# ende76/brotli-rs

Hardware: AMD Instinct MI355X
Metric: decompressed MB/s (whole node), alice29x4096 batch (higher is better)
Workload: dtype u8; 1 GPU; 4096 x alice29.txt.compressed per GPU; streams_per_gpu=4096

## Files before the change

brotli-rs_amd/build.py:

```python
import os
import re
import subprocess
import sys

PKG = os.path.dirname(os.path.abspath(__file__))
ROOT = os.path.dirname(PKG)
CSRC = os.path.join(PKG, "csrc")
LIB_PATH = os.path.join(PKG, "libbrx.so")
HIPCC = os.environ.get("HIPCC", "/opt/rocm/bin/hipcc")
SOURCES = ["brx_kernels.hip", "brx_kernels_l1.hip", "brx_kernels_l2.hip", "brx_kernels_l3.hip", "brx_kernels_l4.hip", "brx_kernels_s.hip", "brx_gen.hip", "brx_util.hip", "brx_tiles.hip", "brx_digest.hip", "brx_index.hip", "brx_api.cpp", "brx_node.cpp"]
DEPS = SOURCES + ["brx_device.h", "brx_layout.h", "brx_tiles.h", "brx_digest.h", "brx_index.h", "brx_internal.h", "brx_plan.h", "brx_small.h", "brx_hot.S", "brx_lens.S", os.path.join("..", "host", "brx_walk.cpp"), os.path.join("..", "..", "include", "brx.h"),
                  os.path.join("..", "tables", "dictionary.bin"), os.path.join("..", "tables", "context_lut.bin"),
                  os.path.join("..", "tables", "transforms.bin"), os.path.join("..", "tables", "gen_header.bin"), os.path.join("..", "build.py")]


def _stale():
    if not os.path.exists(LIB_PATH):
        return True
    t = os.path.getmtime(LIB_PATH)
    return any(os.path.getmtime(os.path.join(CSRC, d)) > t for d in DEPS)


def build_library(force=False, verbose=False):
    if not force and not _stale():
        return LIB_PATH
    import fcntl
    with open(os.path.join(PKG, ".build.lock"), "w") as lock:
        fcntl.flock(lock, fcntl.LOCK_EX)
        if not force and not _stale():
            return LIB_PATH
        return _build_locked(verbose)


def _build_locked(verbose):
    if not os.path.exists(HIPCC):
        if os.path.exists(LIB_PATH):
            return LIB_PATH
        raise RuntimeError("hipcc not found at %s and no prebuilt libbrx.so" % HIPCC)
    gen = os.path.join(CSRC, "_gen", "brx_tables_gen.h")
    subprocess.check_call([sys.executable, os.path.join(ROOT, "tools", "bin2h.py"), gen, "BRX", "static const"])
    prof = ["-DBRX_PROF"] if os.environ.get("BRX_PROF") == "1" else []
    if os.environ.get("BRX_NO_SPEC") == "1":
        prof.append("-DBRX_NO_SPEC")
    if os.environ.get("BRX_PIN_NOPS"):
        prof.append("-DPIN_NOPS=%d" % int(os.environ["BRX_PIN_NOPS"]))
    extra = ["-D" + d for d in os.environ.get("BRX_DEFS", "").split()]
    prof += extra
    instances = [("" if k == 0 else "_l%d" % k, "-DBRX_LEVEL=%d" % k) for k in range(5)] + [("_s", "-DBRX_SMALL")]

    def emit(src, name, defs):
        txt = subprocess.check_output(["cpp", "-P", "-x", "assembler-with-cpp"] + defs + [os.path.join(CSRC, src)]).decode()
        assert ")BRXASM" not in txt and "%" not in txt and "{" not in txt and "$" not in txt
        if src == "brx_hot.S":
            if "-DBRX_WIN_SGPR" in defs:
                txt = txt.replace(".L", ".LS_")
            macros = re.findall(r"^\s*\.macro\s+(\w+)", txt, flags=re.M)
            txt += "".join(".purgem %s\n" % m for m in macros)
        else:
            txt = re.sub(r"@(\d+)@", r"%\1", txt).replace(".Lls_", ".Lls%=_")
        with open(os.path.join(CSRC, "_gen", name), "w") as f:
            f.write("// generated from %s by build.py -- do not edit\n" % src)
            f.write('R"BRXASM(\n' + txt + ')BRXASM"\n')

    for suffix, level in instances:
        if suffix != "_s":
            emit("brx_hot.S", "brx_hot_asm%s.h" % suffix, prof + [level])
            emit("brx_hot.S", "brx_hot_asm_sw%s.h" % suffix, prof + [level, "-DBRX_WIN_SGPR"])
        emit("brx_lens.S", "brx_lens_asm%s.h" % suffix, [level])
    cmd = [HIPCC, "--offload-arch=gfx950", "-O3", "-std=c++17", "-fPIC", "-shared", "-Wno-comment"]
    if os.environ.get("BRX_BRINGUP") == "1" or os.environ.get("BRX_PROF") == "1":
        cmd.append("-DBRX_BRINGUP")
    cmd += extra + [os.path.join(CSRC, s) for s in SOURCES]
    tmp = "%s.tmp.%d" % (LIB_PATH, os.getpid())
    cmd += ["-ldl", "-lpthread", "-o", tmp]
    if verbose:
        print(" ".join(cmd))
    subprocess.check_call(cmd, cwd=CSRC)
    os.replace(tmp, LIB_PATH)
    walk = os.path.join(PKG, "brx_walk")
    subprocess.check_call(["g++", "-O2", "-std=c++17", os.path.join(PKG, "host", "brx_walk.cpp"), "-o", walk + ".tmp", "-L", PKG,
                           "-lbrx", "-Wl,-rpath,$ORIGIN", "-Wl,-rpath,/opt/rocm/lib", "-L/opt/rocm/lib", "-lamdhip64"])
    os.replace(walk + ".tmp", walk)
    return LIB_PATH


if __name__ == "__main__":
    print(build_library(force="--force" in sys.argv, verbose=True))
```

brotli-rs_amd/csrc/brx_kernels.hip:

```cpp
#include <hip/hip_runtime.h>

#include "brx_device.h"

#ifdef BRX_SMALL
#define BRX_INST _s
#elif BRX_LEVEL == 0
#define BRX_INST
#else
#define BRX_INST BRX_L_PASTE(_l, BRX_LEVEL)
#endif
#define BRX_NAME(stem) BRX_L_PASTE(stem, BRX_INST)
#define BRX_STR_(x) #x
#define BRX_STR(x) BRX_STR_(x)
#define BRX_GEN_H(stem) BRX_STR(_gen/BRX_NAME(stem).h)

typedef unsigned char u8;
typedef unsigned short u16;
typedef unsigned int u32;
typedef unsigned long long u64;

#define RMASK (BRX_RING_BYTES - 1u)
#define TM_BYTES (BRX_TM_WORDS * 4u)

enum {
// ... 250 lines not shown
        d.chunkA = in_load_chunk(d, d.cbase);
        d.chunkB = in_load_chunk(d, d.cbase + 64u);
    }
    while (w >= d.cbase + 128u) {
        d.chunkA = d.chunkB;
        d.cbase += 64u;
        d.chunkB = in_load_chunk(d, d.cbase + 64u);
    }
    u32 k = w - d.cbase;
    return k < 64u ? rdl(d.chunkA, k) : rdl(d.chunkB, k - 64u);
}
FI void in_seek(Dec &d, u64 bitpos) {
    d.bitpos = bitpos;
    d.ww = (u32)(bitpos >> 5);
    u64 lo = in_word(d, d.ww);
    u64 hi = in_word(d, d.ww + 1u);
    d.win = lo | (hi << 32);
}
FI u64 in_remaining(const Dec &d) { return d.bitend - d.bitpos; }
FI u32 in_peek_raw(const Dec &d) { return (u32)(d.win >> (d.bitpos & 31u)); }
FI void in_consume(Dec &d, u32 n) {
    d.bitpos += n;
    if ((u32)(d.bitpos >> 5) != d.ww) {
        d.ww += 1u;
        u64 hi = in_word(d, d.ww + 1u);
        d.win = (d.win >> 32) | (hi << 32);
    }
}
FI bool in_bits(Dec &d, u32 n, u32 &v) {
    if (in_remaining(d) < n) return false;
    v = n ? (in_peek_raw(d) & ((1u << n) - 1u)) : 0u;
    in_consume(d, n);
    return true;
}
FI u32 in_byte_tail(Dec &d) {
    u32 k = (u32)(d.bitpos & 7u);
    u32 v = 0;
    if (k) in_bits(d, 8u - k, v);
    return v;
}

#define ST_STARTED 33
#define ST_ISLAST 34
#define ST_MLEN 35
#define ST_IACTAB 36
#define ST_POOL 38
#define ST_MIRROR 40
#define ST_PAUSE_AT 43
#define ST_IN_LOW 45
#define ST_SPEC 47
#define ST_NEED 42
#define SEG_NEED_HEADER 100u
#define SEG_PAUSED 101u
#define HC_WHOLE 0u
#define HC_START 1u
#define HC_RESUME_R0 2u
#define HC_RESUME_R1 3u
#define HC_RESUME_R2 4u
#define HC_RESUME_R1_WHOLE 5u
#define HC_TO_END 8u
#define HC_CONTINUE 200u
#define MBW_ASM 31
#define MBW_MBLEFT 32
#define MBW_INS 33
#define MBW_CPY 34
#define MBW_IZ 35
#define MBW_DIST 36
#define MBW_DISTBAD 37
#define MBW_EXIT 38
#define BRX_END_MARGIN 5u
#ifndef BRX_SPEC_CK_DWORDS
#define BRX_SPEC_CK_DWORDS 64u
#endif
#ifndef BRX_SPEC_CK_MIN_DWORDS
#define BRX_SPEC_CK_MIN_DWORDS 1024u
#endif
#define MBW_WSAFE 39

#ifndef BRX_SMALL
FI void put64(Lds &s, u32 i, u64 v) { s.st[i] = (u32)v; s.st[i + 1u] = (u32)(v >> 32); }
FI u64 get64(const Lds &s, u32 i) { return (u64)rfl(s.st[i]) | ((u64)rfl(s.st[i + 1u]) << 32); }
FI void dec_store(const Dec &d, Lds &s) {
    {
        put64(s, 0, (u64)(uintptr_t)d.in_words); s.st[2] = d.w_end; put64(s, 3, d.bitpos); put64(s, 5, d.bitend);
        put64(s, 7, (u64)(uintptr_t)d.out); s.st[9] = d.cap; s.st[10] = d.pos; s.st[11] = d.a; s.st[12] = d.vfl;
        s.st[13] = d.window; s.st[14] = d.dist0; s.st[15] = d.dist1; s.st[16] = d.dist2; s.st[17] = d.dist3;
        s.st[18] = d.lds_top; s.st[19] = d.scr_top; put64(s, 20, (u64)(uintptr_t)d.scratch); s.st[22] = d.needed;
        put64(s, 23, (u64)(uintptr_t)d.t_dict); put64(s, 25, (u64)(uintptr_t)d.t_xforms);
        put64(s, 27, (u64)(uintptr_t)d.t_lut); put64(s, 29, d.wd); put64(s, 31, d.wd_limit);
        put64(s, ST_POOL, (u64)(uintptr_t)d.pool);
        put64(s, ST_MIRROR, (u64)(uintptr_t)d.mirror);
    }
}
FI void dec_load(Dec &d, const Lds &s) {
    d.lane = threadIdx.x;
    d.in_words = (const u32 *)(uintptr_t)get64(s, 0); d.w_end = rfl(s.st[2]);
    d.bitend = get64(s, 5);
    d.out = (u8 *)(uintptr_t)get64(s, 7); d.cap = rfl(s.st[9]);
    d.out_rsrc = __builtin_amdgcn_make_buffer_rsrc(d.out, 0, d.cap, 0x00020000);
    d.mirror = (u8 *)(uintptr_t)get64(s, ST_MIRROR);
    d.out2_rsrc = __builtin_amdgcn_make_buffer_rsrc(d.mirror, 0, d.mirror ? d.cap : 0u, 0x00020000);
    d.pos = rfl(s.st[10]); d.a = rfl(s.st[11]);
    d.vfl = rfl(s.st[12]); d.window = rfl(s.st[13]);
    d.dist0 = rfl(s.st[14]); d.dist1 = rfl(s.st[15]); d.dist2 = rfl(s.st[16]); d.dist3 = rfl(s.st[17]);
    d.lds_top = rfl(s.st[18]); d.scr_top = rfl(s.st[19]); d.scratch = (u32 *)(uintptr_t)get64(s, 20);
    d.needed = rfl(s.st[22]);
    d.t_dict = (const u8 *)(uintptr_t)get64(s, 23); d.t_xforms = (const BrxTransform *)(uintptr_t)get64(s, 25);
    d.t_lut = (const u32 *)(uintptr_t)get64(s, 27); d.wd = get64(s, 29); d.wd_limit = get64(s, 31);
    d.pool = (const BrxSlabPool *)(uintptr_t)get64(s, ST_POOL);
    d.need_cur = 0u; d.need_peak = 0u;
    d.cbase = 0xffffff00u;
    d.chunkA = 0; d.chunkB = 0;
    in_seek(d, get64(s, 3));
}

FI void dec_load_in(Dec &d, const Lds &s) {
    d.lane = threadIdx.x;
    d.in_words = (const u32 *)(uintptr_t)get64(s, 0); d.w_end = rfl(s.st[2]);
    d.bitend = get64(s, 5);
    d.lds_top = rfl(s.st[18]); d.scr_top = rfl(s.st[19]); d.scratch = (u32 *)(uintptr_t)get64(s, 20);
    d.pool = (const BrxSlabPool *)(uintptr_t)get64(s, ST_POOL);
    d.need_cur = 0u; d.need_peak = 0u;
    d.cbase = 0xffffff00u;
    d.chunkA = 0; d.chunkB = 0;
    in_seek(d, get64(s, 3));
}
FI void dec_store_in(const Dec &d, Lds &s) {
    put64(s, 3, d.bitpos);
    s.st[18] = d.lds_top; s.st[19] = d.scr_top; put64(s, 20, (u64)(uintptr_t)d.scratch);
    s.st[ST_NEED] = d.need_peak;
}

#endif

#define BRX_HDR_WORDS 17u
#define BRX_HDR_INFO 16u
#define BRX_DIST_UNFIT 0xc0000000u
template <bool INL, bool WIDE> FI u32 decode_sym_as(Dec &d, const Lds &s, u32 h, u32 &sym) {
    u32 hv = tm_ld32<INL>(d, s, h + (d.lane & 31u));
    u32 h0 = rdl(hv, BRX_HDR_INFO);
    u32 kind = h0 & 3u;
    if (kind == 0u) return LK_NONE;
    if (kind == 1u) {
        sym = h0 >> 16;
        if (WIDE && sym == 0xffffu) sym = rfl(tm_ld32<INL>(d, s, h + 13u));
        return LK_OK;
    }
    u64 rem = in_remaining(d);
    u32 peek = in_peek_raw(d) & 0x7fffu;
    if (rem < 15u) peek &= (1u << (u32)rem) - 1u;
    u32 v = __brev(peek) >> 17;
    u64 m = ballot(((v << 16) | 0xffffu) < hv) & 0xfffeull;
    if (m == 0ull) {
        u32 maxlen = (h0 >> 8) & 0xffu;
        return rem >= (u64)(maxlen + 1u) ? LK_NONE : LK_EOF;
    }
    u32 L = (u32)__builtin_ctzll(m);
    if ((u64)L > rem) return LK_EOF;
    u32 base = rdl(hv, L);
    u32 idx = ((v >> (15u - L)) + base) & 0xffffu;
    sym = WIDE ? rfl(tm_ld32<INL>(d, s, h + BRX_HDR_WORDS + idx)) : rfl(tm_ld16<INL>(d, s, (h + BRX_HDR_WORDS) * 2u + idx));
    in_consume(d, L);
    return LK_OK;
}
FI u32 decode_sym(Dec &d, const Lds &s, u32 h, u32 &sym) {
    if (h < BRX_TM_WORDS) return decode_sym_as<true, false>(d, s, h, sym);
    return decode_sym_as<false, false>(d, s, h, sym);
}
FI u32 decode_sym_wide(Dec &d, const Lds &s, u32 h, u32 &sym) {
    if (h < BRX_TM_WORDS) return decode_sym_as<true, true>(d, s, h, sym);
    return decode_sym_as<false, true>(d, s, h, sym);
}

#ifdef BRX_SMALL
FI u32 hb_word(Dec &d, u32 w) {
    const u32 v = rfl(w < 64u ? rdl(d.chunkA, w & 63u) : rdl(d.chunkB, w & 63u));
    return w < 128u ? v : 0u;
}
#else
FI u32 hb_word(Dec &d, u32 w) {
    const u32 v = in_word(d, w);
    return w == d.hb_lastw ? v & d.hb_lastmask : v;
}
#endif
FI void hb_begin(Dec &d) {
    const u32 w = (u32)(d.bitpos >> 5), sh = (u32)d.bitpos & 31u;
    d.hb_lastw = (u32)((d.bitend - 1ull) >> 5);
    const u32 r = (u32)d.bitend & 31u;
    d.hb_lastmask = r ? (1u << r) - 1u : 0xffffffffu;
    const u64 lo = hb_word(d, w), hi = hb_word(d, w + 1u);
    d.win = (lo | (hi << 32)) >> sh;
    d.nav = 64u - sh;
    d.ww = w + 2u;
}
FI u64 hb_pos(const Dec &d) { return 32ull * d.ww - d.nav; }
FI bool hb_over(const Dec &d) { return hb_pos(d) > d.bitend; }
FI u32 hb_peek(const Dec &d) { return (u32)d.win; }
FI void hb_skip(Dec &d, u32 n) {
    d.win >>= n;
    d.nav -= n;
    if (d.nav < 32u) {
        d.win |= (u64)hb_word(d, d.ww) << d.nav;
        d.nav += 32u;
        d.ww += 1u;
    }
}
FI u32 hb_bits(Dec &d, u32 n) {
    const u32 v = hb_peek(d) & ((1u << n) - 1u);
    hb_skip(d, n);
    return v;
}

FI u32 row_scan_add(u32 x) {
    x += (u32)__builtin_amdgcn_update_dpp(0, (int)x, 0x111, 0xf, 0xf, true);
    x += (u32)__builtin_amdgcn_update_dpp(0, (int)x, 0x112, 0xf, 0xf, true);
    x += (u32)__builtin_amdgcn_update_dpp(0, (int)x, 0x114, 0xf, 0xf, true);
    x += (u32)__builtin_amdgcn_update_dpp(0, (int)x, 0x118, 0xf, 0xf, true);
    return x;
}
FI u32 lanes_below(u64 m) { return __builtin_amdgcn_mbcnt_hi((u32)(m >> 32), __builtin_amdgcn_mbcnt_lo((u32)m, 0u)); }

FI u32 emit_code_header(Dec &d, Lds &s, u32 cnt, const bool wide, u32 &off) {
    const u32 lane = d.lane, L = lane & 15u;
    const u32 c = (lane - 1u) < 15u ? cnt : 0u;
    const u32 lim = row_scan_add(c << (15u - L));
    const u32 offi = row_scan_add(c);
    off = offi - c;
    const u32 base = off - ((lim >> (15u - L)) - c);
    const u32 nnz = rdl(offi, 15);
    const u32 maxlen = 63u - (u32)__builtin_clzll(ballot(c != 0u) | 1ull);
    const u32 h = tm_alloc(d, BRX_HDR_WORDS + (wide ? nnz : ((nnz + 1u) >> 1)));
    const u32 w = lane == 0u ? 0u : lane == BRX_HDR_INFO ? (2u | (maxlen << 8) | (nnz << 16)) : (lim << 16) | (base & 0xffffu);
    if (h < BRX_TM_WORDS) { if (lane < BRX_HDR_WORDS) tm_st32<true>(d, s, h + lane, w); }
    else { if (lane < BRX_HDR_WORDS) tm_st32<false>(d, s, h + lane, w); }
    return h;
}
FI void code_put_symbol(const Dec &d, Lds &s, u32 h, const bool wide, bool on, u32 slot, u32 sym) {
    if (wide) {
        if (h < BRX_TM_WORDS) { if (on) tm_st32<true>(d, s, h + BRX_HDR_WORDS + slot, sym); }
        else { if (on) tm_st32<false>(d, s, h + BRX_HDR_WORDS + slot, sym); }
    } else {
        if (h < BRX_TM_WORDS) { if (on) tm_st16<true>(d, s, (h + BRX_HDR_WORDS) * 2u + slot, sym); }
        else { if (on) tm_st16<false>(d, s, (h + BRX_HDR_WORDS) * 2u + slot, sym); }
    }
}

FI u32 build_code(Dec &d, Lds &s, u32 n, const bool wide = false) {
    const u32 lane = d.lane;
    u32 *const cnt = (u32 *)&s.lens[704];
    if (lane < 16u) cnt[lane] = 0u;
    const u32 nch = (n + 63u) >> 6;
    for (u32 c = 0; c < nch; c++) {
        const u32 i = c * 64u + lane;
        const u32 my = i < n ? s.lens[i] : 0u;
        __hip_atomic_fetch_add(&cnt[my], 1u, __ATOMIC_RELAXED, __HIP_MEMORY_SCOPE_WORKGROUP);
    }
    u32 off;
    const u32 h = emit_code_header(d, s, cnt[lane & 15u], wide, off);
    if (lane < 16u) cnt[lane] = off;
    for (u32 c = 0; c < nch; c++) {
        const u32 i = c * 64u + lane;
        const u32 my = i < n ? s.lens[i] : 0u;
        if (ballot(my != 0u) == 0ull) continue;
        const u64 b0 = ballot((my & 1u) != 0u), b1 = ballot((my & 2u) != 0u), b2 = ballot((my & 4u) != 0u), b3 = ballot((my & 8u) != 0u);
        u64 eq = (my & 1u) ? b0 : ~b0;
        eq &= (my & 2u) ? b1 : ~b1;
        eq &= (my & 4u) ? b2 : ~b2;
        eq &= (my & 8u) ? b3 : ~b3;
        const u32 slot = cnt[my] + lanes_below(eq);
        code_put_symbol(d, s, h, wide, my != 0u, slot, i);
        __hip_atomic_fetch_add(&cnt[my], 1u, __ATOMIC_RELAXED, __HIP_MEMORY_SCOPE_WORKGROUP);
    }
    return h;
}

FI u32 build_simple(Dec &d, Lds &s, u32 nsym, u32 k0, u32 k1, u32 k2, u32 k3, const bool wide) {
    if (nsym < 3u) k2 = 0xffffffffu;
    if (nsym < 4u) k3 = 0xffffffffu;
    u32 t;
#define BRX_CSWAP(a, b) do { t = a < b ? a : b; b = a < b ? b : a; a = t; } while (0)
    BRX_CSWAP(k0, k1); BRX_CSWAP(k2, k3); BRX_CSWAP(k0, k2); BRX_CSWAP(k1, k3); BRX_CSWAP(k1, k2);
#undef BRX_CSWAP
    const u32 lane = d.lane;
    const u32 cnt = (u32)((k0 >> 16) == lane) + (u32)((k1 >> 16) == lane) + (u32)((k2 >> 16) == lane) + (u32)((k3 >> 16) == lane);
    u32 off;
    const u32 h = emit_code_header(d, s, cnt, wide, off);
    const u32 mine = lane == 0u ? k0 : lane == 1u ? k1 : lane == 2u ? k2 : k3;
    code_put_symbol(d, s, h, wide, lane < nsym, lane, mine & 0xffffu);
    return h;
}

FI u32 build_single(Dec &d, Lds &s, u32 sym) {
    u32 h = tm_alloc(d, BRX_HDR_WORDS);
    u32 w = d.lane == BRX_HDR_INFO ? (1u | (sym << 16)) : 0u;
    if (h < BRX_TM_WORDS) { if (d.lane < BRX_HDR_WORDS) tm_st32<true>(d, s, h + d.lane, w); }
    else { if (d.lane < BRX_HDR_WORDS) tm_st32<false>(d, s, h + d.lane, w); }
    return h;
}

FI void lens_clear(const Dec &d, Lds &s, u32 n) {
    for (u32 i = d.lane * 4u; i < n; i += 256u) *(u32 *)&s.lens[i] = 0u;
}

FI u32 read_complex_lens(Dec &d, Lds &s, u32 hskip, u32 alphabet) {
    PT_BEGIN(pt);
    const u32 lane = d.lane;
    u32 clv = 0;
    u32 sum = 0, nonzero = 0, single = 0;
    bool parallel_done = false;
#ifndef BRX_NO_PAR_CLCODE
    {
        const u32 w0 = hb_word(d, d.ww), w1 = hb_word(d, d.ww + 1u);
        const u64 lo = d.nav < 64u ? (d.win | ((u64)w0 << d.nav)) : d.win;
        const u64 hi = ((u64)w0 >> (64u - d.nav)) | ((u64)w1 << (d.nav - 32u));
        const u32 p = (u32)((lo >> lane) | (lane ? hi << ((64u - lane) & 63u) : 0ull)) & 15u;
        const u32 len = (p & 1u) == 0u ? 2u : (p & 2u) == 0u ? 2u : (p & 4u) == 0u ? 3u : 4u;
        const u32 val = (p & 1u) == 0u ? ((p & 2u) ? 3u : 0u) : (p & 2u) == 0u ? 4u : (p & 4u) == 0u ? 2u : ((p & 8u) ? 5u : 1u);
        const u32 lv = len | (val << 4);
        const u32 nx = lane + len;
        const u32 j1 = nx < 63u ? nx : 63u;
        const u32 j2 = (u32)__shfl((int)j1, (int)j1), j4 = (u32)__shfl((int)j2, (int)j2), j8 = (u32)__shfl((int)j4, (int)j4),
                  j16 = (u32)__shfl((int)j8, (int)j8);
        u32 pos = 0;
        {
            const u32 t1 = (u32)__shfl((int)j1, (int)pos); pos = (lane & 1u) ? t1 : pos;
            const u32 t2 = (u32)__shfl((int)j2, (int)pos); pos = (lane & 2u) ? t2 : pos;
            const u32 t4 = (u32)__shfl((int)j4, (int)pos); pos = (lane & 4u) ? t4 : pos;
            const u32 t8 = (u32)__shfl((int)j8, (int)pos); pos = (lane & 8u) ? t8 : pos;
            const u32 t16 = (u32)__shfl((int)j16, (int)pos); pos = (lane & 16u) ? t16 : pos;
        }
        const u32 mine = (u32)__shfl((int)lv, (int)pos);
        const u32 n = 18u - hskip;
        const u32 myval = lane < n ? mine >> 4 : 0u, mylen = mine & 15u;
        const u32 space = myval ? 32u >> myval : 0u;
        const u32 sc = row_scan_add(space);
        const u32 cum = lane >= 16u ? sc + rdl(sc, 15) : sc;
        const u64 hit = ballot(lane < n && cum >= 32u);
        const u32 count = hit ? (u32)__builtin_ctzll(hit) + 1u : n;
        const u32 last_end = rdl(pos + mylen, count - 1u);
        if (last_end <= 60u) {
            sum = rdl(cum, count - 1u);
            const u64 nzm = ballot(lane < count && myval != 0u);
            nonzero = (u32)__builtin_popcountll(nzm);
            const u32 inv = lane == 0u ? 4u : lane <= 4u ? lane - 1u : lane == 5u ? 5u : lane == 6u ? 7u : lane == 16u ? 8u : lane == 17u ? 6u : lane + 2u;
            const u32 k = inv - hskip;
            const u32 got = (u32)__shfl((int)myval, (int)(k & 63u));
            clv = (lane < 18u && k < count) ? got : 0u;
            if (nzm) {
                const u32 kl = 63u - (u32)__builtin_clzll(nzm), il = hskip + kl;
                single = il < 4u ? il + 1u : il == 4u ? 0u : il == 5u ? 5u : il == 6u ? 17u : il == 7u ? 6u : il == 8u ? 16u : il - 2u;
            }
            hb_skip(d, last_end > 32u ? 32u : last_end);
            if (last_end > 32u) hb_skip(d, last_end - 32u);
            if (sum > 32u) return ST_CODE_LENGTHS_CHECKSUM;
            parallel_done = true;
        }
    }
#endif
    for (u32 i = hskip; i < 18u && !parallel_done; i++) {
        const u32 p = hb_peek(d) & 15u;
        u32 len, val;
        if ((p & 1u) == 0u) { len = 2; val = (p & 2u) ? 3u : 0u; }
        else if ((p & 2u) == 0u) { len = 2; val = 4u; }
        else if ((p & 4u) == 0u) { len = 3; val = 2u; }
        else { len = 4; val = (p & 8u) ? 5u : 1u; }
        hb_skip(d, len);
        if (val) {
            const u32 symi = i < 4u ? i + 1u : i == 4u ? 0u : i == 5u ? 5u : i == 6u ? 17u : i == 7u ? 6u : i == 8u ? 16u : i - 2u;
            clv = wrl(val, symi, clv);
            sum += 32u >> val;
            nonzero++;
            single = symi;
            if (sum == 32u) break;
            if (sum > 32u) return ST_CODE_LENGTHS_CHECKSUM;
        }
    }
    if (nonzero == 0u) return ST_NO_CODE_LENGTH;
    if (nonzero >= 2u && sum < 32u) return ST_CODE_LENGTHS_CHECKSUM;

    u32 cltab = 0;
    if (nonzero >= 2u) {
        const u32 l = lane < 18u ? clv : 0u;
        const u64 b0 = ballot((l & 1u) != 0u), b1 = ballot((l & 2u) != 0u), b2 = ballot((l & 4u) != 0u);
        u64 eq = (l & 1u) ? b0 : ~b0;
        eq &= (l & 2u) ? b1 : ~b1;
        eq &= (l & 4u) ? b2 : ~b2;
        const u32 rank = lanes_below(eq);
        u32 code = 0, mycode = 0;
        for (u32 k = 1; k <= 5u; k++) {
            if (l == k) mycode = code + rank;
            const u64 mk = ((k & 1u) ? b0 : ~b0) & ((k & 2u) ? b1 : ~b1) & ((k & 4u) ? b2 : ~b2);
            code = (code + (u32)__builtin_popcountll(mk)) << 1;
        }
        const u32 rev = l ? __brev(mycode) >> (32u - l) : 0u;
        u64 todo = ballot(l != 0u);
        while (todo) {
            const u32 sy = (u32)__builtin_ctzll(todo);
            todo &= todo - 1ull;
            const u32 ls = rdl(l, sy), rs = rdl(rev, sy);
            if ((lane & ((1u << ls) - 1u)) == rs) cltab = (sy << 4) | ls;
        }
    }

    lens_clear(d, s, alphabet);
    PT_ADD(7, pt);
    u32 total = 0, i = 0, nz = 0;
    u32 last_symbol = 0xffu, last_repeat = 0, last_nz = 8;
    u32 cur = 0;
    bool dirty = false;
#define BRX_LENS_FLUSH(base_) do { if (dirty) s.lens[(base_) + lane] = (u8)cur; cur = 0u; dirty = false; } while (0)
    if (nonzero >= 2u) {
        u32 stat, nz_a, i_a, dirty_a, cur_a, vt0, vt1;
        u64 win = (u64)rfl((u32)d.win) | ((u64)rfl((u32)(d.win >> 32)) << 32);
        u32 nav = rfl(d.nav), ww = rfl(d.ww), cbase = rfl(d.cbase), cha = d.chunkA, chb = d.chunkB;
        asm volatile(
#include BRX_GEN_H(brx_lens_asm)
            : "=s"(stat), "=s"(nz_a), "=s"(i_a), "=s"(dirty_a), "+s"(win), "+s"(nav), "+s"(ww), "+s"(cbase), "+v"(cha), "+v"(chb),
              "=&v"(cur_a), "=&v"(vt0), "=&v"(vt1)
            : "s"(alphabet), "s"(d.w_end), "s"(d.hb_lastw), "s"(d.hb_lastmask), "s"((u64)(uintptr_t)d.in_words), "v"(cltab), "v"(lane)
            : "memory", "vcc", "scc", "s60", "s61", "s62", "s63", "s64", "s65", "s66", "s67", "s68", "s69", "s70", "s71", "s72", "s73",
              "s74", "s75", "s76", "s77", "s78", "s79", "s80", "s81", "s82", "s83", "s84", "s85", "s86", "s87", "s88", "s89", "s90");
        d.win = win; d.nav = nav; d.ww = ww; d.cbase = cbase; d.chunkA = cha; d.chunkB = chb;
        if (dirty_a) s.lens[((i_a - 1u) & ~63u) + lane] = (u8)cur_a;
        PT_ADD(8, pt);
        if (stat) return stat;
        if (nz_a < 2u) return ST_LESS_THAN_TWO_NONZERO;
        return ST_OK;
    }
    while (i < alphabet) {
        u32 sym;
        if (nonzero == 1u) {
            sym = single;
        } else {
            const u32 e = rdl(cltab, hb_peek(d) & 31u);
            sym = e >> 4;
            hb_skip(d, e & 15u);
        }
        if (sym <= 15u) {
            cur = wrl(sym, i & 63u, cur);
            i++;
            last_symbol = sym;
            last_repeat = 0;
            if (sym) {
                dirty = true;
                nz++;
                last_nz = sym;
                total += 32768u >> sym;
                if (total == 32768u) break;
                if (total > 32768u) return ST_CODE_LENGTHS_CHECKSUM;
            }
            if ((i & 63u) == 0u) BRX_LENS_FLUSH(i - 64u);
        } else if (sym == 16u) {
            const u32 v = hb_bits(d, 2);
            u32 add, new_repeat;
            if (last_symbol == 16u && last_repeat) {
                new_repeat = 4u * (last_repeat - 2u) + v + 3u;
                add = new_repeat - last_repeat;
            } else {
                new_repeat = 3u + v;
                add = new_repeat;
            }
            if (i + add > alphabet) return ST_PARSE_COMPLEX_LENGTHS;
            nz += add;
            total += add * (32768u >> last_nz);
            for (u32 left = add; left != 0u;) {
                const u32 a0 = i & 63u, k = left < 64u - a0 ? left : 64u - a0;
                cur = (lane - a0) < k ? last_nz : cur;
                dirty = true;
                i += k;
                left -= k;
                if ((i & 63u) == 0u) BRX_LENS_FLUSH(i - 64u);
            }
            if (total == 32768u) break;
            if (total > 32768u) return ST_CODE_LENGTHS_CHECKSUM;
            last_repeat = new_repeat;
            last_symbol = 16u;
        } else {
            const u32 v = hb_bits(d, 3);
            u32 ni;
            if (last_symbol == 17u && last_repeat) {
                const u32 new_repeat = 8u * (last_repeat - 2u) + v + 3u;
                ni = i + (new_repeat - last_repeat);
                last_repeat = new_repeat;
            } else {
                last_repeat = 3u + v;
                ni = i + last_repeat;
            }
            if (ni > alphabet) return ST_PARSE_COMPLEX_LENGTHS;
            if ((ni >> 6) != (i >> 6)) BRX_LENS_FLUSH(i & ~63u);
            i = ni;
            last_symbol = 17u;
        }
    }
    BRX_LENS_FLUSH((i - 1u) & ~63u);
#undef BRX_LENS_FLUSH
    PT_ADD(8, pt);
    if (nz < 2u) return ST_LESS_THAN_TWO_NONZERO;
    return ST_OK;
}

FI u32 read_prefix_code(Dec &d, Lds &s, u32 alphabet, u32 &h, const bool wide = false) {
    PT_BEGIN(pt);
    const u32 kind = hb_bits(d, 2);
    if (kind == 1u) {
        const u32 bit_width = 32u - (u32)__builtin_clz(alphabet - 1u);
        const u32 nsym = hb_bits(d, 2) + 1u;
        u32 s0 = 0, s1 = 0, s2 = 0, s3 = 0;
        s0 = hb_bits(d, bit_width);
        if (s0 >= alphabet) return ST_INVALID_SYMBOL;
        if (nsym > 1u) {
            s1 = hb_bits(d, bit_width);
            if (s1 >= alphabet) return ST_INVALID_SYMBOL;
        }
        if (nsym > 2u) {
            s2 = hb_bits(d, bit_width);
            if (s2 >= alphabet) return ST_INVALID_SYMBOL;
        }
        if (nsym > 3u) {
            s3 = hb_bits(d, bit_width);
            if (s3 >= alphabet) return ST_INVALID_SYMBOL;
        }
        if (nsym > 1u && s0 == s1) return ST_INVALID_SYMBOL;
        if (nsym > 2u && (s0 == s2 || s1 == s2)) return ST_INVALID_SYMBOL;
        if (nsym > 3u && (s0 == s3 || s1 == s3 || s2 == s3)) return ST_INVALID_SYMBOL;
        u32 tree_select = 0;
        if (nsym == 4u) tree_select = hb_bits(d, 1);
        if (nsym == 1u) {
            h = build_single(d, s, s0);
            PT_ADD(6, pt);
            return ST_OK;
        }
        u32 l0, l1, l2, l3;
        if (nsym == 2u) { l0 = 1; l1 = 1; l2 = 0; l3 = 0; }
        else if (nsym == 3u) { l0 = 1; l1 = 2; l2 = 2; l3 = 0; }
        else if (!tree_select) { l0 = l1 = l2 = l3 = 2; }
        else { l0 = 1; l1 = 2; l2 = 3; l3 = 3; }
        h = build_simple(d, s, nsym, (l0 << 16) | s0, (l1 << 16) | s1, (l2 << 16) | s2, (l3 << 16) | s3, wide);
        PT_ADD(6, pt);
        return ST_OK;
    }
    const u32 rc = read_complex_lens(d, s, kind, alphabet);
    if (rc) return rc;
    PT_BEGIN(pb);
    h = build_code(d, s, alphabet, wide);
    PT_ADD(9, pb);
    return ST_OK;
}

FI void ring_put(const Dec &d, Lds &s, bool on, u32 vpos, u32 byte) {
    u8 *p = on ? &s.ring[vpos & RMASK] : &s.trash[d.lane];
    *p = (u8)byte;
}
#define OUT_STORE128(q, off) do { const u32 off_ = (off); __builtin_amdgcn_raw_buffer_store_b128((q), d.out_rsrc, off_, 0, 0); \
                                  __builtin_amdgcn_raw_buffer_store_b128((q), d.out2_rsrc, off_, 0, 0); } while (0)
#define OUT_STORE8(b, off) do { const u32 off_ = (off); __builtin_amdgcn_raw_buffer_store_b8((u8)(b), d.out_rsrc, off_, 0, 0); \
                                __builtin_amdgcn_raw_buffer_store_b8((u8)(b), d.out2_rsrc, off_, 0, 0); } while (0)
FI void flush_range(Dec &d, const Lds &s, u32 v0, u32 v1) {
    const u32 u0 = (v0 + 15u) >> 4, u1 = v1 >> 4;
    for (u32 ub = u0; ub < u1; ub += 64u) {
        u32 u = ub + d.lane;
        typedef u32 u32x4 __attribute__((ext_vector_type(4)));
        u32x4 q = *(const u32x4 *)&s.ring[(u * 16u) & RMASK];
        u32 off = u < u1 ? u * 16u - d.a : 0xffffffffu;
        OUT_STORE128(q, off);
    }
    if (v0 & 15u) {
        u32 e = u0 * 16u < v1 ? u0 * 16u : v1;
        u32 v = v0 + d.lane;
        u32 b = s.ring[v & RMASK];
        OUT_STORE8(b, v < e ? v - d.a : 0xffffffffu);
    }
    if ((v1 & 15u) && u1 * 16u >= v0 && u1 >= u0) {
        u32 v = u1 * 16u + d.lane;
        u32 b = s.ring[v & RMASK];
        OUT_STORE8(b, v < v1 ? v - d.a : 0xffffffffu);
    }
    d.vfl = v1;
}
FI void maybe_flush(Dec &d, const Lds &s) {
    u32 vpos = d.pos + d.a;
    for (;;) {
        u32 blk_end = (d.vfl & ~(BRX_FLUSH_BLOCK - 1u)) + BRX_FLUSH_BLOCK;
        if (vpos < blk_end + BRX_FLUSH_LAG) break;
        flush_range(d, s, d.vfl, blk_end);
    }
}
FI bool out_room(Dec &d, u32 n) {
    if ((u64)d.pos + n > (u64)d.cap) {
        d.needed = (u64)d.pos + n > 0xffffffffull ? 0xffffffffu : d.pos + n;
        return false;
    }
    return true;
}
FI void ctx_bytes(const Dec &d, const Lds &s, u32 &p1, u32 &p2) {
    u32 v = d.pos + d.a;
    u32 b1 = s.ring[(v - 1u) & RMASK], b2 = s.ring[(v - 2u) & RMASK];
    p1 = d.pos >= 1u ? rfl(b1) : 0u;
    p2 = d.pos >= 2u ? rfl(b2) : 0u;
}

FI u32 copy_fetch(const Dec &d, const Lds &s, u32 back_max, u32 back_min, u32 back) {
    if (back_max <= BRX_RING_BYTES) return s.ring[(d.pos - back + d.a) & RMASK];
    if (back_min > BRX_RING_BYTES) return __builtin_amdgcn_raw_buffer_load_b8(d.out_rsrc, d.pos - back, 0, 0);
    u32 bn = s.ring[(d.pos - back + d.a) & RMASK];
    u32 bf = __builtin_amdgcn_raw_buffer_load_b8(d.out_rsrc, d.pos - back, 0, 0);
    return back <= BRX_RING_BYTES ? bn : bf;
}

typedef u32 u32x4 __attribute__((ext_vector_type(4)));
FI void bulk_copy_1k(Dec &d, Lds &s, u32 de) {
    const u32 vdst = d.pos + d.a + 16u * d.lane;
    u32x4 q;
    if (de <= BRX_RING_BYTES) {
        const u32 r = vdst - de;
        if ((de & 3u) == 0u) {
            q.x = *(const u32 *)&s.ring[r & RMASK];
            q.y = *(const u32 *)&s.ring[(r + 4u) & RMASK];
            q.z = *(const u32 *)&s.ring[(r + 8u) & RMASK];
            q.w = *(const u32 *)&s.ring[(r + 12u) & RMASK];
        } else {
            u32 w[4];
            _Pragma("unroll") for (u32 k = 0; k < 4u; k++) {
                u32 b0 = s.ring[(r + 4u * k) & RMASK], b1 = s.ring[(r + 4u * k + 1u) & RMASK];
                u32 b2 = s.ring[(r + 4u * k + 2u) & RMASK], b3 = s.ring[(r + 4u * k + 3u) & RMASK];
                w[k] = b0 | (b1 << 8) | (b2 << 16) | (b3 << 24);
            }
            q.x = w[0]; q.y = w[1]; q.z = w[2]; q.w = w[3];
        }
    } else {
        q = __builtin_amdgcn_raw_buffer_load_b128(d.out_rsrc, d.pos - de + 16u * d.lane, 0, 0);
    }
    *(u32x4 *)&s.ring[vdst & RMASK] = q;
    d.pos += 1024u;
}

#ifndef BRX_FILL_AUX
#define BRX_FILL_AUX 0
#endif
FI void periodic_fill(Dec &d, Lds &s, u32 P, u32 nblocks) {
    flush_range(d, s, d.vfl, d.pos + d.a);
    const u32 base = d.pos - P + d.a;
    u32 o = (16u * d.lane) % P;
    const u32 step = 1024u % P;
    {
        u32x4 q = *(const u32x4 *)&s.ring[(base + o) & RMASK];
        u32 off = d.pos + 16u * d.lane;
        if (step == 0u) {
            if (d.mirror == nullptr) {
                for (u32 k = 0; k < nblocks; k++) { __builtin_amdgcn_raw_buffer_store_b128(q, d.out_rsrc, off, 0, BRX_FILL_AUX); off += 1024u; }
            } else {
                for (u32 k = 0; k < nblocks; k++) { OUT_STORE128(q, off); off += 1024u; }
            }
        } else {
            const bool both = d.mirror != nullptr;
            for (u32 k = 0; k < nblocks; k++) {
                o += step;
                o = o >= P ? o - P : o;
                const u32x4 qn = *(const u32x4 *)&s.ring[(base + o) & RMASK];
                __builtin_amdgcn_raw_buffer_store_b128(q, d.out_rsrc, off, 0, BRX_FILL_AUX);
                if (both) __builtin_amdgcn_raw_buffer_store_b128(q, d.out2_rsrc, off, 0, 0);
                off += 1024u;
                q = qn;
            }
        }
        d.pos += nblocks << 10;
    }
    d.vfl = d.pos + d.a;
    static_assert(BRX_RING_BYTES == 2048u, "periodic_fill re-seeds two 1 KiB blocks");
    if (nblocks >= 2u) {
        const u32 o1 = o >= step ? o - step : o + P - step;
        const u32 o0 = o1 >= step ? o1 - step : o1 + P - step;
        const u32x4 q0 = *(const u32x4 *)&s.ring[(base + o0) & RMASK];
        const u32x4 q1 = *(const u32x4 *)&s.ring[(base + o1) & RMASK];
        const u32 off = d.pos - BRX_RING_BYTES + 16u * d.lane;
        *(u32x4 *)&s.ring[(off + d.a) & RMASK] = q0;
        *(u32x4 *)&s.ring[(off + 1024u + d.a) & RMASK] = q1;
        return;
    }
    __builtin_amdgcn_s_waitcnt(0x0F70);
    for (u32 j = 0; j < BRX_RING_BYTES / 1024u; j++) {
        const u32 off = d.pos - BRX_RING_BYTES + 1024u * j + 16u * d.lane;
        const u32x4 q = __builtin_amdgcn_raw_buffer_load_b128(d.out_rsrc, off, 0, 0);
        *(u32x4 *)&s.ring[(off + d.a) & RMASK] = q;
    }
}

FI void direct_far_copy(Dec &d, Lds &s, u32 de, u32 nblocks) {
    flush_range(d, s, d.vfl, d.pos + d.a);
    for (u32 k = 0; k < nblocks; k++) {
        if (de < 16384u) __builtin_amdgcn_s_waitcnt(0x0F70);
        const u32 src = d.pos - de + 16u * d.lane, dst = d.pos + 16u * d.lane;
        const u32x4 q0 = __builtin_amdgcn_raw_buffer_load_b128(d.out_rsrc, src, 0, 0);
        const u32x4 q1 = __builtin_amdgcn_raw_buffer_load_b128(d.out_rsrc, src + 1024u, 0, 0);
        const u32x4 q2 = __builtin_amdgcn_raw_buffer_load_b128(d.out_rsrc, src + 2048u, 0, 0);
        const u32x4 q3 = __builtin_amdgcn_raw_buffer_load_b128(d.out_rsrc, src + 3072u, 0, 0);
        OUT_STORE128(q0, dst);
        OUT_STORE128(q1, dst + 1024u);
        OUT_STORE128(q2, dst + 2048u);
        OUT_STORE128(q3, dst + 3072u);
        d.pos += 4096u;
    }
    d.vfl = d.pos + d.a;
    __builtin_amdgcn_s_waitcnt(0x0F70);
    for (u32 j = 0; j < BRX_RING_BYTES / 1024u; j++) {
        const u32 off = d.pos - BRX_RING_BYTES + 1024u * j + 16u * d.lane;
        const u32x4 q = __builtin_amdgcn_raw_buffer_load_b128(d.out_rsrc, off, 0, 0);
        *(u32x4 *)&s.ring[(off + d.a) & RMASK] = q;
    }
}

FI void window_copy(Dec &d, Lds &s, u32 dist, u32 len, u32 &p1, u32 &p2) {
    u32 done = 0, de = dist;
    bool bulk_used = false;
    const u32 g16 = dist & (0u - dist) & 15u ? (dist & (0u - dist) & 15u) : 16u;
    const u32 P16 = dist * (16u / g16);
    while (done < len) {
        const u32 rem = len - done;
        if (dist < len && rem >= 8192u && P16 <= 1024u && done + dist >= P16 && ((d.pos + d.a) & 15u) == 0u) {
            const u32 nb = rem >> 10;
            periodic_fill(d, s, P16, nb);
            done += nb << 10;
            bulk_used = true;
// ... 1428 lines not shown
```

brotli-rs_amd/csrc/brx_lens.S:

```
#include "brx_layout.h"
#define LDS_LENS BRX_L_LENS
#define WIN s[60:61]
#define WINLO s60
#define NAV s62
#define WW s63
#define IPOS s64
#define TOT s65
#define NZ s66
#define LNZ s67
#define LSYM s68
#define LREP s69
#define ALPHA s70
#define CBASE s71
#define WEND s72
#define LASTW s73
#define LMASK s74
#define ENT s75
#define SYM s76
#define LEN s77
#define T0 s78
#define T1 s79
#define PAIR s[80:81]
#define PLO s80
#define PHI s81
#define T2 s82
#define T3 s83
#define LINK s[84:85]
#define INW s[86:87]
#define STAT s88
#define DIRTY s89
#define LEFT s90
#define VCHA @8@
#define VCHB @9@
#define VCUR @10@
#define VT0 @11@
#define VT1 @12@
#define VCLTAB @18@
#define VLANE @19@

    s_mov_b64 WIN, @4@
    s_mov_b32 NAV, @5@
    s_mov_b32 WW, @6@
    s_mov_b32 CBASE, @7@
    s_mov_b32 ALPHA, @13@
    s_mov_b32 WEND, @14@
    s_mov_b32 LASTW, @15@
    s_mov_b32 LMASK, @16@
    s_mov_b64 INW, @17@
    s_mov_b32 IPOS, 0
    s_mov_b32 TOT, 0
    s_mov_b32 NZ, 0
    s_mov_b32 LNZ, 8
    s_mov_b32 LSYM, 0xff
    s_mov_b32 LREP, 0
    s_mov_b32 DIRTY, 0
    s_mov_b32 STAT, 0
    v_mov_b32 VCUR, 0
.Lls_sym:
    s_cmp_ge_u32 IPOS, ALPHA
    s_cbranch_scc1 .Lls_done
    s_and_b32 T0, WINLO, 31
    v_readlane_b32 ENT, VCLTAB, T0
    s_and_b32 LEN, ENT, 15
    s_lshr_b32 SYM, ENT, 4
    s_lshr_b64 WIN, WIN, LEN
    s_sub_u32 NAV, NAV, LEN
    s_cmp_lt_u32 NAV, 32
    s_cbranch_scc0 .Lls_have
    s_call_b64 LINK, .Lls_refill
.Lls_have:
    s_cmp_gt_u32 SYM, 15
    s_cbranch_scc1 .Lls_special
    s_and_b32 T0, IPOS, 63
    v_mov_b32 VT0, SYM
    v_cmp_eq_u32 vcc, T0, VLANE
    v_cndmask_b32 VCUR, VCUR, VT0, vcc
    s_add_u32 IPOS, IPOS, 1
    s_mov_b32 LSYM, SYM
    s_mov_b32 LREP, 0
    s_cmp_eq_u32 SYM, 0
    s_cbranch_scc1 .Lls_chunk
    s_mov_b32 DIRTY, 1
    s_add_u32 NZ, NZ, 1
    s_mov_b32 LNZ, SYM
    s_lshr_b32 T1, 0x8000, SYM
    s_add_u32 TOT, TOT, T1
    s_cmp_ge_u32 TOT, 0x8000
    s_cbranch_scc1 .Lls_total
.Lls_chunk:
    s_and_b32 T0, IPOS, 63
    s_cmp_lg_u32 T0, 0
    s_cbranch_scc1 .Lls_sym
    s_sub_u32 T0, IPOS, 64
    s_call_b64 LINK, .Lls_flush
    s_branch .Lls_sym
.Lls_total:
    s_cmp_eq_u32 TOT, 0x8000
    s_cbranch_scc1 .Lls_done
    s_mov_b32 STAT, 1
    s_branch .Lls_done
.Lls_special:
    s_cmp_eq_u32 SYM, 16
    s_cbranch_scc1 .Lls_rep
    s_and_b32 T0, WINLO, 7
    s_lshr_b64 WIN, WIN, 3
    s_sub_u32 NAV, NAV, 3
    s_cmp_lt_u32 NAV, 32
    s_cbranch_scc0 .Lls_z_have
    s_call_b64 LINK, .Lls_refill
.Lls_z_have:
    s_cmp_eq_u32 LSYM, 17
    s_cselect_b32 T1, LREP, 0
    s_cmp_eq_u32 T1, 0
    s_cbranch_scc1 .Lls_z_fresh
    s_sub_u32 T2, T1, 2
    s_lshl_b32 T2, T2, 3
    s_add_u32 T2, T2, T0
    s_add_u32 T2, T2, 3
    s_sub_u32 T3, T2, T1
    s_mov_b32 LREP, T2
    s_branch .Lls_z_go
.Lls_z_fresh:
    s_add_u32 T3, T0, 3
    s_mov_b32 LREP, T3
.Lls_z_go:
    s_mov_b32 LSYM, 17
    s_add_u32 T2, IPOS, T3
    s_cmp_gt_u32 T2, ALPHA
    s_cbranch_scc1 .Lls_err_parse
    s_xor_b32 T0, T2, IPOS
    s_cmp_lt_u32 T0, 64
    s_cbranch_scc1 .Lls_z_same
    s_and_b32 T0, IPOS, 0xffffffc0
    s_mov_b32 LEFT, T2
    s_call_b64 LINK, .Lls_flush
    s_mov_b32 T2, LEFT
.Lls_z_same:
    s_mov_b32 IPOS, T2
    s_branch .Lls_sym
.Lls_rep:
    s_and_b32 T0, WINLO, 3
    s_lshr_b64 WIN, WIN, 2
    s_sub_u32 NAV, NAV, 2
    s_cmp_lt_u32 NAV, 32
    s_cbranch_scc0 .Lls_r_have
    s_call_b64 LINK, .Lls_refill
.Lls_r_have:
    s_cmp_eq_u32 LSYM, 16
    s_cselect_b32 T1, LREP, 0
    s_cmp_eq_u32 T1, 0
    s_cbranch_scc1 .Lls_r_fresh
    s_sub_u32 T2, T1, 2
    s_lshl_b32 T2, T2, 2
    s_add_u32 T2, T2, T0
    s_add_u32 T2, T2, 3
    s_sub_u32 LEFT, T2, T1
    s_branch .Lls_r_go
.Lls_r_fresh:
    s_add_u32 T2, T0, 3
    s_mov_b32 LEFT, T2
.Lls_r_go:
    s_add_u32 T3, IPOS, LEFT
    s_cmp_gt_u32 T3, ALPHA
    s_cbranch_scc1 .Lls_err_parse
    s_add_u32 NZ, NZ, LEFT
    s_lshr_b32 T3, 0x8000, LNZ
    s_mul_i32 T3, T3, LEFT
    s_add_u32 TOT, TOT, T3
    s_mov_b32 LREP, T2
    s_mov_b32 LSYM, 16
    v_mov_b32 VT1, LNZ
.Lls_r_fill:
    s_and_b32 T0, IPOS, 63
    s_sub_u32 T1, 64, T0
    s_min_u32 T1, T1, LEFT
    v_subrev_u32 VT0, T0, VLANE
    v_cmp_gt_u32 vcc, T1, VT0
    v_cndmask_b32 VCUR, VCUR, VT1, vcc
    s_mov_b32 DIRTY, 1
    s_add_u32 IPOS, IPOS, T1
    s_sub_u32 LEFT, LEFT, T1
    s_and_b32 T0, IPOS, 63
    s_cmp_lg_u32 T0, 0
    s_cbranch_scc1 .Lls_r_next
    s_sub_u32 T0, IPOS, 64
    s_call_b64 LINK, .Lls_flush
    v_mov_b32 VT1, LNZ
.Lls_r_next:
    s_cmp_lg_u32 LEFT, 0
    s_cbranch_scc1 .Lls_r_fill
    s_cmp_ge_u32 TOT, 0x8000
    s_cbranch_scc1 .Lls_total
    s_branch .Lls_sym
.Lls_err_parse:
    s_mov_b32 STAT, 18
    s_branch .Lls_done

.Lls_flush:
    s_cmp_eq_u32 DIRTY, 0
    s_cbranch_scc1 .Lls_flush_empty
    v_add_u32 VT0, T0, VLANE
    ds_write_b8 VT0, VCUR offset:LDS_LENS
.Lls_flush_empty:
    v_mov_b32 VCUR, 0
    s_mov_b32 DIRTY, 0
    s_setpc_b64 LINK

.Lls_refill:
    s_sub_u32 T1, WW, CBASE
    s_cmp_lt_u32 T1, 128
    s_cbranch_scc1 .Lls_rf_staged
    s_waitcnt vmcnt(0)
    v_mov_b32 VCHA, VCHB
    s_add_u32 CBASE, CBASE, 64
    s_add_u32 T1, CBASE, 64
    v_add_u32 VT0, T1, VLANE
    v_cmp_gt_u32 vcc, WEND, VT0
    s_sub_u32 T2, WEND, 1
    v_min_u32 VT1, T2, VT0
    v_lshlrev_b32 VT1, 2, VT1
    global_load_dword VCHB, VT1, INW
    s_waitcnt vmcnt(0)
    v_cndmask_b32 VCHB, 0, VCHB, vcc
    s_sub_u32 T1, WW, CBASE
.Lls_rf_staged:
    s_cmp_lt_u32 T1, 64
    s_cbranch_scc0 .Lls_rf_b
    v_readlane_b32 PLO, VCHA, T1
    s_branch .Lls_rf_have
.Lls_rf_b:
    v_readlane_b32 PLO, VCHB, T1
.Lls_rf_have:
    s_cmp_lt_u32 WW, WEND
    s_cselect_b32 PLO, PLO, 0
    s_cmp_eq_u32 WW, LASTW
    s_cselect_b32 T2, LMASK, -1
    s_and_b32 PLO, PLO, T2
    s_mov_b32 PHI, 0
    s_lshl_b64 PAIR, PAIR, NAV
    s_or_b64 WIN, WIN, PAIR
    s_add_u32 NAV, NAV, 32
    s_add_u32 WW, WW, 1
    s_setpc_b64 LINK

.Lls_done:
    s_mov_b32 @0@, STAT
    s_mov_b32 @1@, NZ
    s_mov_b32 @2@, IPOS
    s_mov_b32 @3@, DIRTY
    s_mov_b64 @4@, WIN
    s_mov_b32 @5@, NAV
    s_mov_b32 @6@, WW
    s_mov_b32 @7@, CBASE
```

Measured before the change: 75820 MB/s.

## Decode complex code-length symbols in parallel across wavefront lanes before serial fallback

```diff
diff --git a/brotli-rs_amd/build.py b/brotli-rs_amd/build.py
--- a/brotli-rs_amd/build.py
+++ b/brotli-rs_amd/build.py
@@ -9,7 +9,7 @@
 LIB_PATH = os.path.join(PKG, "libbrx.so")
 HIPCC = os.environ.get("HIPCC", "/opt/rocm/bin/hipcc")
 SOURCES = ["brx_kernels.hip", "brx_kernels_l1.hip", "brx_kernels_l2.hip", "brx_kernels_l3.hip", "brx_kernels_l4.hip", "brx_kernels_s.hip", "brx_gen.hip", "brx_util.hip", "brx_tiles.hip", "brx_digest.hip", "brx_index.hip", "brx_api.cpp", "brx_node.cpp"]
-DEPS = SOURCES + ["brx_device.h", "brx_layout.h", "brx_tiles.h", "brx_digest.h", "brx_index.h", "brx_internal.h", "brx_plan.h", "brx_small.h", "brx_hot.S", "brx_lens.S", os.path.join("..", "host", "brx_walk.cpp"), os.path.join("..", "..", "include", "brx.h"),
+DEPS = SOURCES + ["brx_device.h", "brx_layout.h", "brx_tiles.h", "brx_digest.h", "brx_index.h", "brx_internal.h", "brx_plan.h", "brx_small.h", "brx_clsyms.h", "brx_hot.S", "brx_lens.S", os.path.join("..", "host", "brx_walk.cpp"), os.path.join("..", "..", "include", "brx.h"),
                   os.path.join("..", "tables", "dictionary.bin"), os.path.join("..", "tables", "context_lut.bin"),
                   os.path.join("..", "tables", "transforms.bin"), os.path.join("..", "tables", "gen_header.bin"), os.path.join("..", "build.py")]
 
diff --git a/brotli-rs_amd/csrc/brx_clsyms.h b/brotli-rs_amd/csrc/brx_clsyms.h
--- /dev/null
+++ b/brotli-rs_amd/csrc/brx_clsyms.h
@@ -0,0 +1,88 @@
+#ifndef BRX_CLSYMS_H
+#define BRX_CLSYMS_H
+
+struct ClState {
+    unsigned i, total, nz, last_nz, last_symbol, last_repeat;
+};
+#define CL_STATE_INIT {0u, 0u, 0u, 8u, 0xffu, 0u}
+
+enum {
+    CL_MORE = 0,
+    CL_DONE = 1,
+    CL_ERR_SUM = 2,
+    CL_ERR_RUN = 3,
+    CL_SERIAL = 4
+};
+#define CL_RUN_MAX 32u
+#define CL_REP_CAP 0x100000u
+
+template <class Sink>
+CL_FN unsigned clsyms_batch(ClState &st, unsigned b0, unsigned b1, unsigned b2, CLV cltab, unsigned alphabet, Sink &sink, unsigned &used) {
+    const CLV lane = cl_lane();
+    const CLV sh = lane & 31u;
+    const CLV wlo = cl_sel(lane < 32u, b0, b1), whi = cl_sel(lane < 32u, b1, b2);
+    const CLV p = (wlo >> sh) | ((whi << 1u) << (31u - sh));
+    const CLV ent = cl_shfl(cltab, p & 31u);
+    const CLV len = ent & 15u, sy = ent >> 4;
+    const CLV xb = cl_sel(sy == 16u, 2u, cl_sel(sy == 17u, 3u, 0u));
+    const CLV x = (p >> len) & ((1u << xb) - 1u);
+    const CLV tl = len + xb;
+    const CLV nx = lane + tl;
+    const CLV j1 = cl_sel(nx < 63u, nx, 63u);
+    const CLV packed = tl | (sy << 4) | (x << 9);
+    const CLV j2 = cl_shfl(j1, j1), j4 = cl_shfl(j2, j2), j8 = cl_shfl(j4, j4), j16 = cl_shfl(j8, j8), j32 = cl_shfl(j16, j16);
+    CLV pos = lane & 0u;
+    pos = cl_sel(lane & 1u, cl_shfl(j1, pos), pos);
+    pos = cl_sel(lane & 2u, cl_shfl(j2, pos), pos);
+    pos = cl_sel(lane & 4u, cl_shfl(j4, pos), pos);
+    pos = cl_sel(lane & 8u, cl_shfl(j8, pos), pos);
+    pos = cl_sel(lane & 16u, cl_shfl(j16, pos), pos);
+    pos = cl_sel(lane & 32u, cl_shfl(j32, pos), pos);
+    const CLV valid = pos < 63u;
+    const CLV me = cl_shfl(packed, pos);
+    const CLV end = pos + (me & 15u);
+    const CLV sym = cl_sel(valid, (me >> 4) & 31u, 0u), fresh = (me >> 9) + 3u;
+    const CLV spec = sym >= 16u, rsh = (sym - 14u) & 3u;
+    const CLV chained = spec & (cl_up1(sym, st.last_repeat ? st.last_symbol : 0xffu) == sym);
+    CLV rep = cl_sel(spec, fresh, 0u);
+    CLV known = chained == 0u;
+    while (cl_ballot(known == 0u)) {
+        const CLV now = (known == 0u) & cl_up1(known, 1u);
+        const CLV r = ((cl_up1(rep, st.last_repeat) - 2u) << rsh) + fresh;
+        rep = cl_sel(now, cl_sel(r < CL_REP_CAP, r, CL_REP_CAP), rep);
+        known = known | now;
+    }
+    const CLV cnt = cl_sel(spec, cl_sel(chained, rep - cl_up1(rep, st.last_repeat), rep), valid);
+    const CLV plain_nz = (sym - 1u) < 15u, is16 = sym == 16u;
+    const CLV src = cl_prev_set(cl_ballot(plain_nz));
+    const CLV lnz = cl_sel(src < 64u, cl_shfl(sym, src & 63u), st.last_nz);
+    const CLV capped = cl_sel(cnt < 2048u, cnt, 2048u);
+    const CLV space = cl_sel(plain_nz, 32768u >> (sym & 15u), cl_sel(is16, capped * (32768u >> (lnz & 15u)), 0u));
+    const CLV ni = st.i + cl_scan(cnt), ip = ni - cnt;
+    const CLV tt = st.total + cl_scan(space);
+    const CLV nzs = cl_scan(cl_sel(plain_nz, 1u, cl_sel(is16, cnt, 0u)));
+    const CLV fl = cl_sel(is16 & (cnt > CL_RUN_MAX), CL_SERIAL, cl_sel(ni > alphabet, CL_ERR_RUN, cl_sel(tt > 32768u, CL_ERR_SUM,
+                   cl_sel((tt == 32768u) | (ni >= alphabet), CL_DONE, CL_MORE))));
+    const unsigned long long ends = cl_ballot(valid & (fl != 0u));
+    const unsigned kend = ends ? (unsigned)__builtin_ctzll(ends) : (unsigned)__builtin_popcountll(cl_ballot(valid)) - 1u;
+    const unsigned r = ends ? cl_get(fl, kend) : (unsigned)CL_MORE;
+    const unsigned taken = r == CL_SERIAL ? kend : kend + 1u;
+    const unsigned stored = (r == CL_SERIAL || r == CL_ERR_RUN) ? kend : kend + 1u;
+    const CLV st_on = lane < stored;
+    cl_store(sink, st_on & plain_nz, ip, sym);
+    const CLV run_on = st_on & is16;
+    for (unsigned t = 0; cl_ballot(run_on & (cnt > t)); t++) cl_store(sink, run_on & (cnt > t), ip + t, lnz);
+    used = 0u;
+    if (taken) {
+        const unsigned e = taken - 1u;
+        st.i = cl_get(ni, e);
+        st.total = cl_get(tt, e);
+        st.nz += cl_get(nzs, e);
+        st.last_nz = cl_get(cl_sel(plain_nz, sym, lnz), e);
+        st.last_symbol = cl_get(sym, e);
+        st.last_repeat = cl_get(rep, e);
+        used = cl_get(end, e);
+    }
+    return r;
+}
+#endif
diff --git a/brotli-rs_amd/csrc/brx_kernels.hip b/brotli-rs_amd/csrc/brx_kernels.hip
--- a/brotli-rs_amd/csrc/brx_kernels.hip
+++ b/brotli-rs_amd/csrc/brx_kernels.hip
@@ -576,6 +576,25 @@
     for (u32 i = d.lane * 4u; i < n; i += 256u) *(u32 *)&s.lens[i] = 0u;
 }
 
+#if !defined(BRX_NO_PAR_CLSYMS) && !defined(BRX_SMALL)
+#define CLV u32
+#define CL_FN FI
+FI u32 cl_lane() { return threadIdx.x; }
+FI u32 cl_sel(u32 c, u32 a, u32 b) { return c ? a : b; }
+FI u32 cl_shfl(u32 v, u32 idx) { return (u32)__shfl((int)v, (int)idx); }
+FI u32 cl_up1(u32 v, u32 first) { const u32 t = (u32)__shfl((int)v, (int)((threadIdx.x - 1u) & 63u)); return threadIdx.x ? t : first; }
+FI u64 cl_ballot(u32 c) { return ballot(c != 0u); }
+FI u32 cl_prev_set(u64 m) { const u64 b = m & ((1ull << threadIdx.x) - 1ull); return b ? 63u - (u32)__builtin_clzll(b) : 64u; }
+FI u32 cl_scan(u32 x) {
+    x = row_scan_add(x);
+    const u32 r0 = rdl(x, 15), r1 = rdl(x, 31), r2 = rdl(x, 47), lane = threadIdx.x;
+    return x + (lane >= 16u ? r0 : 0u) + (lane >= 32u ? r1 : 0u) + (lane >= 48u ? r2 : 0u);
+}
+FI u32 cl_get(u32 v, u32 k) { return rdl(v, k); }
+FI void cl_store(Lds &s, u32 c, u32 i, u32 v) { if (c) s.lens[i] = (u8)v; }
+#include "brx_clsyms.h"
+#endif
+
 FI u32 read_complex_lens(Dec &d, Lds &s, u32 hskip, u32 alphabet) {
     PT_BEGIN(pt);
     const u32 lane = d.lane;
@@ -684,14 +703,42 @@
     bool dirty = false;
 #define BRX_LENS_FLUSH(base_) do { if (dirty) s.lens[(base_) + lane] = (u8)cur; cur = 0u; dirty = false; } while (0)
     if (nonzero >= 2u) {
-        u32 stat, nz_a, i_a, dirty_a, cur_a, vt0, vt1;
+        u32 stat, nz_a = 0, i_a = 0, dirty_a = 0, cur_a = 0, vt0, vt1;
+        u32 tot_a = 0, lnz_a = 8, lsym_a = 0xffu, lrep_a = 0;
+#if !defined(BRX_NO_PAR_CLSYMS) && !defined(BRX_SMALL)
+        {
+            ClState st = CL_STATE_INIT;
+            u32 r;
+            do {
+                const u32 w0 = hb_word(d, d.ww), w1 = hb_word(d, d.ww + 1u);
+                const u64 lo = d.nav < 64u ? (d.win | ((u64)w0 << d.nav)) : d.win;
+                const u64 hi = ((u64)w0 >> (64u - d.nav)) | ((u64)w1 << (d.nav - 32u));
+                u32 used;
+                r = clsyms_batch(st, rfl((u32)lo), rfl((u32)(lo >> 32)), rfl((u32)hi), cltab, alphabet, s, used);
+                for (used = rfl(used); used > 32u; used -= 32u) hb_skip(d, 32u);
+                hb_skip(d, used);
+            } while (r == CL_MORE);
+            if (r != CL_SERIAL) {
+                PT_ADD(8, pt);
+                if (r == CL_ERR_SUM) return ST_CODE_LENGTHS_CHECKSUM;
+                if (r == CL_ERR_RUN) return ST_PARSE_COMPLEX_LENGTHS;
+                if (st.nz < 2u) return ST_LESS_THAN_TWO_NONZERO;
+                return ST_OK;
+            }
+            nz_a = rfl(st.nz); i_a = rfl(st.i); tot_a = rfl(st.total); lnz_a = rfl(st.last_nz); lsym_a = rfl(st.last_symbol); lrep_a = rfl(st.last_repeat);
+            cur_a = s.lens[(i_a & ~63u) + lane];
+            dirty_a = rfl((i_a & 63u) ? 1u : 0u);
+        }
+#endif
         u64 win = (u64)rfl((u32)d.win) | ((u64)rfl((u32)(d.win >> 32)) << 32);
         u32 nav = rfl(d.nav), ww = rfl(d.ww), cbase = rfl(d.cbase), cha = d.chunkA, chb = d.chunkB;
+        const u64 inp = (u64)(uintptr_t)d.in_words, inw = (u64)rfl((u32)inp) | ((u64)rfl((u32)(inp >> 32)) << 32);
         asm volatile(
 #include BRX_GEN_H(brx_lens_asm)
-            : "=s"(stat), "=s"(nz_a), "=s"(i_a), "=s"(dirty_a), "+s"(win), "+s"(nav), "+s"(ww), "+s"(cbase), "+v"(cha), "+v"(chb),
-              "=&v"(cur_a), "=&v"(vt0), "=&v"(vt1)
-            : "s"(alphabet), "s"(d.w_end), "s"(d.hb_lastw), "s"(d.hb_lastmask), "s"((u64)(uintptr_t)d.in_words), "v"(cltab), "v"(lane)
+            : "=s"(stat), "+s"(nz_a), "+s"(i_a), "+s"(dirty_a), "+s"(win), "+s"(nav), "+s"(ww), "+s"(cbase), "+v"(cha), "+v"(chb),
+              "+v"(cur_a), "=&v"(vt0), "=&v"(vt1)
+            : "s"(rfl(alphabet)), "s"(rfl(d.w_end)), "s"(rfl(d.hb_lastw)), "s"(rfl(d.hb_lastmask)), "s"(inw), "v"(cltab), "v"(lane),
+              "s"(tot_a), "s"(lnz_a), "s"(lsym_a), "s"(lrep_a)
             : "memory", "vcc", "scc", "s60", "s61", "s62", "s63", "s64", "s65", "s66", "s67", "s68", "s69", "s70", "s71", "s72", "s73",
               "s74", "s75", "s76", "s77", "s78", "s79", "s80", "s81", "s82", "s83", "s84", "s85", "s86", "s87", "s88", "s89", "s90");
         d.win = win; d.nav = nav; d.ww = ww; d.cbase = cbase; d.chunkA = cha; d.chunkB = chb;
diff --git a/brotli-rs_amd/csrc/brx_lens.S b/brotli-rs_amd/csrc/brx_lens.S
--- a/brotli-rs_amd/csrc/brx_lens.S
+++ b/brotli-rs_amd/csrc/brx_lens.S
@@ -47,15 +47,14 @@
     s_mov_b32 LASTW, @15@
     s_mov_b32 LMASK, @16@
     s_mov_b64 INW, @17@
-    s_mov_b32 IPOS, 0
-    s_mov_b32 TOT, 0
-    s_mov_b32 NZ, 0
-    s_mov_b32 LNZ, 8
-    s_mov_b32 LSYM, 0xff
-    s_mov_b32 LREP, 0
-    s_mov_b32 DIRTY, 0
+    s_mov_b32 IPOS, @2@
+    s_mov_b32 TOT, @20@
+    s_mov_b32 NZ, @1@
+    s_mov_b32 LNZ, @21@
+    s_mov_b32 LSYM, @22@
+    s_mov_b32 LREP, @23@
+    s_mov_b32 DIRTY, @3@
     s_mov_b32 STAT, 0
-    v_mov_b32 VCUR, 0
 .Lls_sym:
     s_cmp_ge_u32 IPOS, ALPHA
     s_cbranch_scc1 .Lls_done
```

After: 75950 MB/s, median of 6. Within noise of the previous version (+0.2%).
